# zkeown/mlx-audio-primitives

Measured on AMD Instinct MI355X. Metric: mel-spectrogram frames/sec (n_fft=2048, n_mels=128), higher is better.
Workload: dtype f32

## Files before the change

### mlx-audio-primitives_amd/csrc/ap_launch.h

```cpp
#pragma once
#include <cstdio>

#include <cstdlib>
#include "../../include/audioprims.h"
#include "ap_common.h"
#include "ap_wave_params.h"

char *ap_error_buffer();

#define AP_FAIL(code, ...)                                         \
    do {                                                           \
        std::snprintf(ap_error_buffer(), 512, __VA_ARGS__);        \
        return (code);                                             \
    } while (0)

static const int64_t kApMaxGrid = 2147483647LL;
static const int64_t kApStreamGrid = 256 * 8;

static inline int ap_grid_1d(int64_t total, int block, int64_t cap) {
    int64_t g = (total + block - 1) / block;
    if (g < 1) g = 1;
    if (g > cap) g = cap;
    return (int)g;
}
// ... 220 lines not shown
                                     const int32_t *desc, int n_waves, int x_complex, int partial_off,
                                     int *n_pass, int *grid) {
    if (P.n_mels > 128 || desc[12] > 256 || desc[15] > 4) return 1;
    if (P.T > (1 << 24) || P.L > (1 << 28)) return 1;
    W.y = P.y;
    W.window = P.window;
    W.tw = P.tw;
    W.parts = plan + desc[11];
    W.n_parts = desc[12];
    W.quads = reinterpret_cast<const float *>(plan + desc[13]);
    W.n_quads = desc[14];
    W.n_slots = desc[7];
    W.hopj = P.hop == 512 ? 4 : 0;
    W.max_row_parts = desc[15];
    W.partial_stride = 0;
    if (partial_off + W.n_slots + 4 > 2 * x_complex || partial_off + 64 > 2 * x_complex) return 1;
    W.rowstart = plan + desc[10];
    W.out = P.out_mel;
    W.max_key = nullptr;
    W.L = P.L;
    W.T = P.T;
    W.Ts = P.T;
    W.tiles_per_clip = 0;
    W.n_tiles = 0;
    W.n_clips = B;
    W.hop = P.hop;
    W.pad = P.pad;
    W.pad_mode = P.pad_mode;
    W.n_mels = P.n_mels;
    W.power = P.power;
    const int pass = (W.n_parts + 63) / 64;
    if (pass < 1 || pass > 4 || W.n_quads < 256 * pass) return 1;
    *n_pass = pass;
    int off = n_waves * x_complex * (int)sizeof(ap_float2);
    W.off_tw2 = off; off += APM_TW2_COMPLEX * (int)sizeof(ap_float2);
    W.off_tw1 = off; off += APM_TW1_COMPLEX * (int)sizeof(ap_float2);
    W.off_win = off; off += APW_NC * (int)sizeof(ap_float2);
    W.off_wq = off; off += ap_align16(W.n_quads * 16);
    W.off_parts = off;
    W.off_partial = 0;
    W.off_otile = 0;
    W.otile_stride = 0;
    W.lds_bytes = off;
    if (off > AP_LDS_MAX) return 1;
    const int64_t n_frames = B * P.T;
    int64_t g = (n_frames + (int64_t)n_waves * 8 - 1) / ((int64_t)n_waves * 8);
    if (g > 256) g = 256;
    if (g < 1) g = 1;
    *grid = (int)g;
    return AP_OK;
}

static inline int ap_prepare_spec_run(ApSpecWaveParams &W, const ApStftParams &P, int64_t B, int n_waves,
                                      int x_complex, int *grid) {
    if (P.plan.n != 2048 || !ap_clip_loads_ok(P)) return 1;
    if (P.T > (1 << 24) || P.L > (1 << 28)) return 1;
    W.y = P.y;
    W.window = P.window;
    W.tw = P.tw;
    W.L = P.L;
    W.T = P.T;
    W.n_clips = B;
    W.hop = P.hop;
    W.pad = P.pad;
    W.hopj = P.hop == 512 ? 4 : 0;
    int off = n_waves * x_complex * (int)sizeof(ap_float2);
    W.off_tw2 = off; off += APM_TW2_COMPLEX * (int)sizeof(ap_float2);
    W.off_tw1 = off; off += APM_TW1_COMPLEX * (int)sizeof(ap_float2);
    W.off_win = off; off += APW_NC * (int)sizeof(ap_float2);
    W.lds_bytes = off;
// ... 691 lines not shown
```

### mlx-audio-primitives_amd/csrc/ap_wave_params.h

```cpp
#pragma once
#include "ap_common.h"

#define APW_NC 1024
#define APW_G 8
#define APW_WAVES 8
#define APW_T1(r) ((r) * 20 + ((r) >> 4) * 2)
#define APW_X_COMPLEX 1284
#define APW_PASSES 4
#define APW_TW2_COMPLEX 72
#define APM_TW_ROW 18
#define APM_TW2_ROW 14
#define APM_TW1_COMPLEX (64 * APM_TW_ROW)
#define APM_TW2_COMPLEX (64 * APM_TW2_ROW)

struct ApMelWaveParams {
    const float *y;
    const float *window;
    const ap_float2 *tw;
    const int32_t *parts;
    const float *quads;
    const int32_t *rowstart;
    float *out;
    unsigned *max_key;
    int64_t L, T, tiles_per_clip, n_tiles, n_clips;
    int64_t Ts;
    int hop, pad, pad_mode, n_mels, n_parts, n_quads, n_slots;
    int hopj;
    int max_row_parts;
    int partial_stride;
    float power;
    int off_tw2, off_tw1, off_win, off_wq, off_parts, off_partial, off_otile, lds_bytes;
    int otile_stride;
};

struct ApSpecWaveParams {
    const float *y;
    const float *window;
    const ap_float2 *tw;
    const float *freq;
    float *centroid, *bandwidth, *rolloff, *flatness;
    int64_t L, T, n_clips;
    int hop, pad, hopj, norm;
    float power, p, roll_percent, amin;
    int off_tw2, off_tw1, off_win, lds_bytes;
};

#define APS_WAVES 8
#define APS_OB_ROW 9
#define APS_OB_ROWS 257

struct ApStftWaveParams {
    const float *y;
    const float *window;
    const ap_float2 *tw;
    ap_float2 *out;
    int64_t L, T, groups_per_clip, n_groups;
    int hop, pad, pad_mode;
    int off_tw2, off_tw1, off_win, off_ob, lds_bytes;
};

#define APS16_G 16
// ... 42 lines not shown
```

### mlx-audio-primitives_amd/csrc/audioprims.hip

```cpp
#include <hip/hip_runtime.h>
#include <cstdlib>
#include <mutex>

#include <cstdio>
#include <cstring>

#include "ap_launch.h"
#include "ap_tu.h"
#include "kernels_generic.h"
#include "kernels_wave.h"
#include "kernels_pointwise.h"
#include "kernels_bigfft.h"
#include "kernels_ct.h"
#include "kernels_wave512.h"
#include "kernels_mel2048.h"
#include "kernels_frames8.h"
#include "kernels_features.h"

static thread_local char g_err[512] = "";

char *ap_error_buffer() { return g_err; }

void ap_set_error(const char *msg) { std::snprintf(g_err, sizeof(g_err), "%s", msg); }

static int ap_check_launch(const char *what) {
    hipError_t e = hipGetLastError();
    if (e != hipSuccess) AP_FAIL(AP_ERR_HIP, "%s: %s", what, hipGetErrorString(e));
    return AP_OK;
}

template <class K>
static int ap_allow_lds(K kernel, int bytes) {
    if (bytes > 48 * 1024) {
        hipError_t e = hipFuncSetAttribute(reinterpret_cast<const void *>(kernel),
                                           hipFuncAttributeMaxDynamicSharedMemorySize, bytes);
        if (e != hipSuccess)
            AP_FAIL(AP_ERR_HIP, "hipFuncSetAttribute(LDS=%d): %s", bytes, hipGetErrorString(e));
    }
    return AP_OK;
}

template <int PMODE, int PADGEN>
static int ap_launch_mel_wave(const ApMelWaveParams &W, int grid, void *stream) {
    int rc = ap_allow_lds(ap_mel2048_wave_kernel<PMODE, PADGEN>, W.lds_bytes);
    if (rc != AP_OK) return rc;
    hipLaunchKernelGGL((ap_mel2048_wave_kernel<PMODE, PADGEN>), dim3(grid), dim3(64 * APW_WAVES), W.lds_bytes,
                       (hipStream_t)stream, W);
    return ap_check_launch("ap_melspec_f32(wave)");
}

template <int PMODE, int HOPJ, int IN16>
static int ap_launch_mel_run_h(const ApMelWaveParams &W, int n_pass, int grid, void *stream) {
#define AP_RUN_LAUNCH(NP)                                                                                \
    do {                                                                                                 \
        int rc = ap_allow_lds(ap_mel2048_run_kernel<PMODE, NP, HOPJ, IN16>, W.lds_bytes);                \
        if (rc != AP_OK) return rc;                                                                      \
        hipLaunchKernelGGL((ap_mel2048_run_kernel<PMODE, NP, HOPJ, IN16>), dim3(grid), dim3(64 * APM_WAVES), \
                           W.lds_bytes, (hipStream_t)stream, W);                                         \
    } while (0)
    if (n_pass == 1) AP_RUN_LAUNCH(1);
    else if (n_pass == 2) AP_RUN_LAUNCH(2);
    else if (n_pass == 3) AP_RUN_LAUNCH(3);
    else AP_RUN_LAUNCH(4);
#undef AP_RUN_LAUNCH
    return ap_check_launch("ap_melspec_f32(run)");
}
template <int PMODE, int IN16 = 0>
static int ap_launch_mel_run(const ApMelWaveParams &W, int n_pass, int grid, void *stream) {
    return W.hopj == 4 ? ap_launch_mel_run_h<PMODE, 4, IN16>(W, n_pass, grid, stream)
                       : ap_launch_mel_run_h<PMODE, 0, IN16>(W, n_pass, grid, stream);
}

static const unsigned kApKeyMinusInf = 0x007FFFFFu;

template <int EPI, int PADGEN>
static int ap_launch_ct(ApStftParams &P, int n_fft, int64_t B, void *stream, bool *handled) {
    *handled = false;
    if (P.L > (1 << 28)) return AP_OK;
    int G = 0, lds = 0;
    *handled = false;
    if (!ap_ct_config(n_fft, EPI == 1 ? P.n_parts : 0, EPI == 1 ? P.n_quads : 0, P.n_mels, &G, &lds)) return AP_OK;
    P.tiles_per_clip = (P.T + G - 1) / G;
    int64_t tiles = P.tiles_per_clip * B;
    const int per_cu = AP_LDS_MAX / lds < 8 ? AP_LDS_MAX / lds : 8;
    int64_t grid = tiles < 256 * per_cu ? tiles : 256 * per_cu;
    int rc = AP_OK;
#define AP_CT_LAUNCH(NC, R0, R1, R2, GG, NT)                                                             \
    do {                                                                                                 \
        rc = ap_allow_lds(ap_stft_ct_kernel<EPI, NC, R0, R1, R2, GG, PADGEN, NT>, lds);                  \
        if (rc != AP_OK) return rc;                                                                      \
        hipLaunchKernelGGL((ap_stft_ct_kernel<EPI, NC, R0, R1, R2, GG, PADGEN, NT>), dim3((unsigned)grid), \
                           dim3(NT), lds, (hipStream_t)stream, P);                                       \
    } while (0)
    if (n_fft == 400) AP_CT_LAUNCH(200, 8, 5, 5, 8, 256);
    else if (n_fft == 512) AP_CT_LAUNCH(256, 16, 16, 1, 8, 256);
    else AP_CT_LAUNCH(512, 16, 8, 4, 8, 256);
#undef AP_CT_LAUNCH
// ... 1210 lines not shown
```

### mlx-audio-primitives_amd/csrc/host_builders.cpp

```cpp
#include <algorithm>
#include <cmath>
#include <cstring>
#include <string>
#include <vector>

#include "../../include/audioprims.h"
#include "ap_common.h"

void ap_set_error(const char *msg);

namespace {

const double kPi = 3.14159265358979323846;

const double F_MIN = 0.0;
const double F_SP = 200.0 / 3.0;
const double MIN_LOG_HZ = 1000.0;
const double MIN_LOG_MEL = (MIN_LOG_HZ - F_MIN) / F_SP;
const double LOGSTEP = std::log(6.4) / 27.0;

double hz_to_mel1(double f, int htk) {
    if (htk) return 2595.0 * std::log10(1.0 + f / 700.0);
    if (f < MIN_LOG_HZ) return (f - F_MIN) / F_SP;
    return MIN_LOG_MEL + std::log(f / MIN_LOG_HZ) / LOGSTEP;
// ... 150 lines not shown
        for (int k = 0; k < F; ++k)
            if (fb[(size_t)m * F + k] != 0.0f) { if (!any) a = k; b = k + 1; any = true; }
        if (!any) continue;
        lo[m] = a;
        len[m] = b - a;
        const int gfirst = a >> 2, glast = (b - 1) >> 2;
        for (int g = gfirst; g <= glast; g += 4) {
            MelPart p;
            p.row = m;
            p.g0 = g;
            p.ng = (glast - g + 1) < 4 ? (glast - g + 1) : 4;
            p.q0 = 0;
            p.slot = (int)parts.size();
            parts.push_back(p);
        }
    }
    std::stable_sort(parts.begin(), parts.end(),
                     [](const MelPart &x, const MelPart &y) { return x.ng > y.ng; });
    int q = 0;
    for (auto &p : parts) { p.q0 = q; q += p.ng; }
}

struct MelWaveLayout {
    std::vector<int> partA, partB;
    int n_quads = 0;
};

const int kB128Groups[4][16] = {
    {0, 1, 2, 3, 12, 13, 14, 15, 20, 21, 22, 23, 24, 25, 26, 27},
    {4, 5, 6, 7, 8, 9, 10, 11, 16, 17, 18, 19, 28, 29, 30, 31},
    {32, 33, 34, 35, 44, 45, 46, 47, 52, 53, 54, 55, 56, 57, 58, 59},
    {36, 37, 38, 39, 40, 41, 42, 43, 48, 49, 50, 51, 60, 61, 62, 63}};

void mel_wave_layout(const std::vector<MelPart> &parts, MelWaveLayout &L) {
    std::vector<std::pair<int, int>> ent;
    size_t i = 0;
    for (; i < parts.size() && parts[i].ng > 2; ++i) ent.push_back({(int)i, -1});
    for (; i < parts.size(); i += 2) ent.push_back({(int)i, i + 1 < parts.size() ? (int)i + 1 : -1});
    const int n = (int)ent.size();
    const int passes = (n + 63) / 64;
    L.partA.assign((size_t)passes * 64, -1);
    L.partB.assign((size_t)passes * 64, -1);
    for (int ps = 0; ps < passes; ++ps) {
        const int first = ps * 64, last = first + 64 < n ? first + 64 : n;
        std::vector<int> bucket[16];
        for (int e = first; e < last; ++e) bucket[parts[ent[e].first].g0 & 15].push_back(e);
        int order[16];
        for (int r = 0; r < 16; ++r) order[r] = r;
        std::stable_sort(order, order + 16, [&](int a, int b) { return bucket[a].size() > bucket[b].size(); });
        std::vector<int> grp[4];
        int has[4][16] = {};
        for (int oi = 0; oi < 16; ++oi) {
            const int r = order[oi];
            for (int idx : bucket[r]) {
                int best = -1;
                for (int g = 0; g < 4; ++g) {
                    if (grp[g].size() >= 16) continue;
                    if (best < 0 || has[g][r] < has[best][r] ||
                        (has[g][r] == has[best][r] && grp[g].size() < grp[best].size()))
                        best = g;
                }
                grp[best].push_back(idx);
                has[best][r]++;
            }
        }
        for (int g = 0; g < 4; ++g)
            for (size_t j = 0; j < grp[g].size(); ++j) {
                const size_t slot = (size_t)ps * 64 + kB128Groups[g][j];
                L.partA[slot] = ent[grp[g][j]].first;
                L.partB[slot] = ent[grp[g][j]].second;
            }
    }
    L.n_quads = passes * 256;
}
}

int64_t ap_mel_plan_words(const float *fb, int n_mels, int n_bins) {
    if (!fb || n_mels <= 0 || n_bins <= 0) return 0;
    std::vector<int> lo, len;
    std::vector<MelPart> parts;
    mel_analyse(fb, n_mels, n_bins, lo, len, parts);
    int64_t quads = 0;
    for (auto &p : parts) quads += p.ng;
    MelWaveLayout L;
    mel_wave_layout(parts, L);
    return 2 * (int64_t)n_mels + 4 * (int64_t)parts.size() + 4 * quads + (int64_t)n_mels + 1 + 8 +
           4 * (int64_t)L.partA.size() + 4 * (int64_t)L.n_quads + 8;
}

int ap_mel_plan_host(const float *fb, int n_mels, int n_bins, int32_t *plan, int32_t *desc) {
    if (!fb || !plan || !desc || n_mels <= 0 || n_bins <= 0) {
        ap_set_error("mel plan: bad arguments");
        return AP_ERR_INVALID;
    }
    const int M = n_mels, F = n_bins;
    std::vector<int> lo, len;
    std::vector<MelPart> parts;
    mel_analyse(fb, M, F, lo, len, parts);
    int64_t quads = 0;
    for (auto &p : parts) quads += p.ng;
    const int64_t words = ap_mel_plan_words(fb, M, F);
    std::memset(plan, 0, sizeof(int32_t) * (size_t)words);
    std::memset(desc, 0, sizeof(int32_t) * AP_PLAN_DESC_INTS);
    int64_t off = 0;
    const int64_t off_lo = off; off += M;
    const int64_t off_len = off; off += M;
    off += off & 3 ? 4 - (off & 3) : 0;
    const int64_t off_parts = off; off += 4 * (int64_t)parts.size();
    const int64_t off_quads = off; off += 4 * quads;
    const int64_t off_rs = off; off += (int64_t)M + 1;
    off += off & 3 ? 4 - (off & 3) : 0;
    MelWaveLayout WL;
    mel_wave_layout(parts, WL);
    const int64_t off_wparts = off; off += 4 * (int64_t)WL.partA.size();
    const int64_t off_wquads = off; off += 4 * (int64_t)WL.n_quads;
    for (int m = 0; m < M; ++m) { plan[off_lo + m] = lo[m]; plan[off_len + m] = len[m]; }
    bool parts_ok = true;
    {
        std::vector<int> cnt(M, 0);
        for (auto &p : parts) cnt[p.row]++;
        int acc = 0;
        for (int m = 0; m < M; ++m) { plan[off_rs + m] = acc; acc += cnt[m]; }
        plan[off_rs + M] = acc;
    }
    float *wq = reinterpret_cast<float *>(plan + off_quads);
    for (size_t i = 0; i < parts.size(); ++i) {
        const MelPart &p = parts[i];
        plan[off_parts + 4 * i + 0] = p.slot;
        plan[off_parts + 4 * i + 1] = p.g0;
        plan[off_parts + 4 * i + 2] = p.ng;
        plan[off_parts + 4 * i + 3] = p.q0;
        for (int g = 0; g < p.ng; ++g)
            for (int e = 0; e < 4; ++e) {
                const int k = 4 * (p.g0 + g) + e;
                wq[4 * (size_t)(p.q0 + g) + e] = k < F ? fb[(size_t)p.row * F + k] : 0.0f;
            }
    }
    float *wwq = reinterpret_cast<float *>(plan + off_wquads);
    int max_row_parts = 0;
    for (int m = 0; m < M; ++m)
        if (plan[off_rs + m + 1] - plan[off_rs + m] > max_row_parts)
            max_row_parts = plan[off_rs + m + 1] - plan[off_rs + m];
    const int32_t dump = (int32_t)parts.size();
    auto put_rows = [&](size_t e, int row0, const MelPart &p, int g_first, int g_count) {
        const size_t col = (e / 64) * 256 + (e % 64);
        for (int g = 0; g < g_count; ++g)
// ... 108 lines not shown
```

### mlx-audio-primitives_amd/csrc/kernels_mel2048.h

```cpp
#pragma once
#include <type_traits>
#include "kernels_wave.h"

#define APM_WAVES 8
#define APM_RUN 8
#define APM_PARTIAL_OFF 1152

#define APM_REG_WIN 1
#define APM_REG_TW1 2
#define APM_REG_TW2 4
#define APM_REG_SPLIT 8
#define APM_REGS (APM_REG_WIN | APM_REG_SPLIT)

AP_DEV int apm_gidx(int g) { return 4 * g + 2 * (g >> 3); }

struct ApmPairLane {
    int L, lp;
    bool l0;
    int rd[4];
};

AP_DEV ApmPairLane apm_pair_lane_init(int lane) {
    ApmPairLane p;
    p.L = apm_lane_index(lane);
// ... 47 lines not shown
        const int a = lane & 3, bq = lane >> 2;
#pragma unroll
        for (int k = 0; k < 16; ++k) X[APW_T1(k * 4 + a) + bq] = v[k];
    }
    AP_WAVE_SYNC();
#pragma unroll
    for (int i = 0; i < 16; ++i) v[i] = X[APW_T1(lane) + i];
    AP_WAVE_SYNC();
    ApButterfly<16>::run_twiddled_fused(v, t1, v);
    if (REGS & APM_REG_TW2) {
#pragma unroll
        for (int i = 0; i < 12; ++i) t2[i] = t2r[i];
    } else {
        apm_load_row(tw2row, t2);
    }
    const int wb = apm_gidx(c.k1p) + (lane & 3);
#pragma unroll
    for (int cc = 0; cc < 16; ++cc) X[wb + 68 * cc] = v[cc];
    AP_WAVE_SYNC();
}

AP_DEV void apm_pair_bins(const ApmPairLane &p, int (&k)[8]) {
    k[0] = p.L; k[1] = p.L + 256; k[2] = 512 - p.lp; k[3] = 256 - p.lp;
    k[4] = p.L + 64; k[5] = p.L + 320; k[6] = 448 - p.L; k[7] = 192 - p.L;
}

AP_DEV void apm_split_twiddles(const ApmPairLane &p, const ap_float2 *tw, ap_float2 (&wsp)[8]) {
    int k[8];
    apm_pair_bins(p, k);
#pragma unroll
    for (int i = 0; i < 8; ++i) wsp[i] = ap_scale(tw[k[i]], 0.5f);
}

template <int PMODE>
AP_DEV void apm_split(const ap_float2 *X, float *pp, const ApmPairLane &p, const ap_float2 (&wsp)[8],
                      const ap_float2 (&t2)[12], const ApwLane &c, float power) {
    ap_float2 z[4][4];
#pragma unroll
    for (int s = 0; s < 4; ++s) {
        const ap_float4 *src = reinterpret_cast<const ap_float4 *>(X + p.rd[s]);
        const ap_float4 lo = src[0], hi = src[1];
        z[s][0] = ap_mk(lo.x, lo.y); z[s][1] = ap_mk(lo.z, lo.w);
        z[s][2] = ap_mk(hi.x, hi.y); z[s][3] = ap_mk(hi.z, hi.w);
    }
    AP_WAVE_SYNC();
#pragma unroll
    for (int s = 0; s < 4; ++s)
        ap_fft4_twiddled3(z[s][0], z[s][1], t2[3 * s], z[s][2], t2[3 * s + 1], z[s][3], t2[3 * s + 2]);
    const ap_float2 zk[8] = {z[0][0], z[0][1], z[3][1], z[3][0], z[1][0], z[1][1], z[2][1], z[2][0]};
    const ap_float2 zm[8] = {p.l0 ? z[0][0] : z[3][3], p.l0 ? z[0][3] : z[3][2], p.l0 ? z[3][2] : z[0][2],
                             p.l0 ? z[3][3] : z[0][3], z[2][3], z[2][2], z[1][2], z[1][3]};
    int k[8];
    apm_pair_bins(p, k);
#pragma unroll
    for (int i = 0; i < 8; ++i) {
        const ap_float2 a = ap_add_conj(zk[i], zm[i]);
        const ap_float2 d = ap_sub_conj(zk[i], zm[i]);
        const ap_float2 u = ap_mul_fw(d, wsp[i]);
        const ap_float2 xk = ap_fma_add_mi(a, c.half, u);
        const ap_float2 xm = ap_fma_sub_mi(a, c.half, u);
        pp[k[i]] = apw_pow2x<PMODE>(xk.x, xk.y, power);
        pp[APW_NC - k[i]] = apw_pow2x<PMODE>(xm.x, xm.y, power);
    }
    if (p.l0) pp[APW_NC / 2] = apw_pow2x<PMODE>(z[0][2].x, z[0][2].y, power);
}

#ifdef AP_DIAG_STAMPS
#define AP_DIAG_BEGIN() unsigned long long ap_dt0, ap_dr0; \
    asm volatile("s_memtime %0\n\ts_memrealtime %1\n\ts_waitcnt lgkmcnt(0)" : "=s"(ap_dt0), "=s"(ap_dr0)::"memory")
#define AP_DIAG_END(widx) do { unsigned long long ap_dt1, ap_dr1; \
    asm volatile("s_memtime %0\n\ts_memrealtime %1\n\ts_waitcnt lgkmcnt(0)" : "=s"(ap_dt1), "=s"(ap_dr1)::"memory"); \
    if ((threadIdx.x & 63) == 0 && (widx) < 256 * 16) { ap_diag_stamps[4 * (widx)] = ap_dt1 - ap_dt0; ap_diag_stamps[4 * (widx) + 1] = ap_dr1 - ap_dr0; ap_diag_stamps[4 * (widx) + 2] = ap_dr0; ap_diag_stamps[4 * (widx) + 3] = ap_dr1; } } while (0)
#else
#define AP_DIAG_BEGIN() do {} while (0)
#define AP_DIAG_END(widx) do {} while (0)
#endif

#ifdef AP_HOST_EMU
#define AP_FAIR_SHARE(wave, nw, f) do {} while (0)
#else
#define AP_FAIR_SHARE(wave, nw, f)                                   \
    do {                                                             \
        if ((wave) >= (nw) / 2 + ((nw) > 8 ? 2 : 0)) {               \
            if ((f) & 1) __builtin_amdgcn_s_setprio(1);              \
            else __builtin_amdgcn_s_setprio(0);                      \
        } else if ((nw) > 8 && (wave) >= 4) {                        \
            if ((f) & 1) __builtin_amdgcn_s_setprio(0);              \
            else __builtin_amdgcn_s_setprio(1);                      \
        }                                                            \
    } while (0)
#endif

template <int PMODE, int NPASS, int HOPJ, int IN16 = 0, int NW = APM_WAVES, int REGS = APM_REGS>
__global__ void __launch_bounds__(64 * NW, NW / 4) ap_mel2048_run_kernel(ApMelWaveParams P) {
    static_assert(IN16 != 1 || (REGS & APM_REG_WIN), "the PCM scale rides on the register-resident window");
    const int tid = threadIdx.x;
    const int lane = tid & 63;
    const int wave = AP_UNIFORM(tid >> 6);
    ap_float2 *X = reinterpret_cast<ap_float2 *>(ap_smem) + wave * APW_X_COMPLEX;
    ap_float2 *TW2 = reinterpret_cast<ap_float2 *>(ap_smem + P.off_tw2);
    const ap_float2 *TW1 = reinterpret_cast<const ap_float2 *>(ap_smem + P.off_tw1);
    const ap_float2 *WIN = reinterpret_cast<const ap_float2 *>(ap_smem + P.off_win);
    const ap_float4 *WQ = reinterpret_cast<const ap_float4 *>(ap_smem + P.off_wq);
    float *pp = reinterpret_cast<float *>(X);
    float *partial = pp + APM_PARTIAL_OFF;
    const int M = P.n_mels;

    {
        const int nt = 64 * NW;
        ap_float4 *wq = reinterpret_cast<ap_float4 *>(ap_smem + P.off_wq);
        for (int i = tid; i < P.n_quads; i += nt) wq[i] = reinterpret_cast<const ap_float4 *>(P.quads)[i];
        apm_fill_tables(TW2, reinterpret_cast<ap_float2 *>(ap_smem + P.off_tw1),
                        reinterpret_cast<ap_float2 *>(ap_smem + P.off_win), P.tw, P.window, tid, nt);
    }
    AP_LDS_BARRIER();
    const ApwLane lc = apw_lane_init(lane, TW2, P.tw, APM_TW_ROW);
    const ApmPairLane pl = apm_pair_lane_init(lane);
    ap_float2 winr[16], t1r[16], t2r[12], wsp[8];
#pragma unroll
    for (int j = 0; j < 16; ++j) {
        winr[j] = (REGS & APM_REG_WIN) ? reinterpret_cast<const ap_float2 *>(P.window)[lane + 64 * j] : ap_mk(0.0f, 0.0f);
        if (IN16 == 1) winr[j] = ap_scale(winr[j], 1.0f / 32768.0f);
        t1r[j] = (REGS & APM_REG_TW1) ? P.tw[2 * (4 * j + (lane & 3)) * (lane >> 2)] : ap_mk(0.0f, 0.0f);
        if (j < 12)
            t2r[j] = (REGS & APM_REG_TW2) ? P.tw[32 * (j % 3 + 1) * (apm_lane_group(pl.L, j / 3) >> 4)] : ap_mk(0.0f, 0.0f);
    }
    apm_split_twiddles(pl, P.tw, wsp);
    const ap_float4 *pqa[NPASS], *pqb[NPASS];
    float *sa[NPASS], *sb[NPASS];
    float fz[NPASS];
#pragma unroll
    for (int ps = 0; ps < NPASS; ++ps) {
        const int pi = lane + 64 * ps;
        ap_int4 pd;
        pd.x = P.n_slots; pd.y = 0; pd.z = P.n_slots; pd.w = 0;
        if (pi < P.n_parts) pd = reinterpret_cast<const ap_int4 *>(P.parts)[pi];
        pqa[ps] = reinterpret_cast<const ap_float4 *>(pp) + pd.y;
        pqb[ps] = reinterpret_cast<const ap_float4 *>(pp) + pd.w;
        sa[ps] = partial + pd.x;
        sb[ps] = partial + (pd.z < 0 ? P.n_slots : pd.z);
        fz[ps] = pd.z < 0 ? 1.0f : 0.0f;
    }
    int rs0[2], cnt[2];
#pragma unroll
    for (int i = 0; i < 2; ++i) {
        const int row = lane + 64 * i;
        rs0[i] = row < M ? P.rowstart[row] : 0;
        cnt[i] = row < M ? P.rowstart[row + 1] - rs0[i] : 0;
    }
    AP_LDS_BARRIER();

    const int64_t worker = (int64_t)blockIdx.x * NW + wave;
    const int64_t n_workers = (int64_t)gridDim.x * NW;
    const int64_t n_frames = P.n_clips * P.T;
    const int64_t f_lo = n_frames * worker / n_workers, f_hi = n_frames * (worker + 1) / n_workers;
    const int Ti = (int)P.T;
    float vmax = -INFINITY;
    AP_DIAG_BEGIN();
    if (f_lo < f_hi) {
        int64_t b = f_lo / P.T;
        int t = (int)(f_lo - b * P.T);
        const int16_t *y16 = reinterpret_cast<const int16_t *>(P.y);
        ApClip clip = ap_clip_make(P.y + (IN16 == 1 ? 0 : b * P.L), IN16 == 1 ? 0 : P.L);
        ApClip16 clip16 = ap_clip16_make(y16 + (IN16 == 1 ? b * P.L : 0), IN16 == 1 ? P.L : 0);
        auto ld2 = [&](int64_t bb, int base, int p) -> ap_float2 {
            if (IN16 == 1) return ap_clip16_load2(clip16, p);
            if (IN16 == 2 && !(base >= 0 && (int64_t)base + 2 * APW_NC <= P.L)) {
                const float *yb = P.y + bb * P.L;
                return ap_mk(ap_load_padded(yb, P.L, p, P.pad_mode), ap_load_padded(yb, P.L, p + 1, P.pad_mode));
            }
            return ap_clip_load2(clip, p);
        };
        constexpr int U = HOPJ == 4 ? 4 : 1;
        ap_float2 raw[16];
        auto load_frame = [&](int tt, auto rot_tag) {
            constexpr int ROT = decltype(rot_tag)::value;
            const int base = tt * P.hop - P.pad;
#pragma unroll
            for (int j = 0; j < 16; ++j) {
                const int p = base + 2 * (lane + 64 * j);
                raw[(j + HOPJ * ROT) & 15] = ld2(b, base, p);
            }
        };
        const int r0 = U == 4 ? (t & 3) : 0;
        if (r0 == 1) load_frame(t, std::integral_constant<int, 1 % U>());
        else if (r0 == 2) load_frame(t, std::integral_constant<int, 2 % U>());
        else if (r0 == 3) load_frame(t, std::integral_constant<int, 3 % U>());
        else load_frame(t, std::integral_constant<int, 0>());
        float acc0[APM_RUN], acc1[APM_RUN];
#pragma unroll
        for (int i = 0; i < APM_RUN; ++i) { acc0[i] = 0.0f; acc1[i] = 0.0f; }
        int nrun = 0, half = U == 4 ? ((t >> 2) & 1) : 0;
        int64_t f = f_lo;

        auto frame = [&](auto rot_tag) -> bool {
            constexpr int ROT = decltype(rot_tag)::value;
            constexpr int NROT = (ROT + 1) % U;
            AP_FAIR_SHARE(wave, NW, f);
            const bool clip_ends = t + 1 == Ti;
            const bool more = f + 1 < f_hi;
            ap_float2 t2[12];
            {
                ap_float2 xs[16], ws[16];
#pragma unroll
                for (int j = 0; j < 16; ++j) xs[j] = raw[(j + HOPJ * ROT) & 15];
                if (REGS & APM_REG_WIN) {
#pragma unroll
                    for (int j = 0; j < 16; ++j) ws[j] = winr[j];
                } else {
#pragma unroll
                    for (int j = 0; j < 16; ++j) ws[j] = WIN[lane + 64 * j];
                }
                AP_SCHED_FENCE();
                apm_forward<REGS>(xs, ws, X, TW1 + APM_TW_ROW * lane, TW2 + APM_TW2_ROW * lane, t1r, t2r, t2, lc);
            }
            AP_SCHED_FENCE();
            if (more) {
                if (clip_ends) {
                    if (IN16 == 1) clip16 = ap_clip16_make(y16 + (b + 1) * P.L, P.L);
                    else clip = ap_clip_make(P.y + (b + 1) * P.L, P.L);
                }
                const int base = (clip_ends ? 0 : t + 1) * P.hop - P.pad;
#pragma unroll
                for (int j = 16 - HOPJ; j < 16; ++j) {
                    const int p = base + 2 * (lane + 64 * j);
                    raw[(j + HOPJ * NROT) & 15] = ld2(clip_ends ? b + 1 : b, base, p);
                }
                if (HOPJ == 0 || clip_ends) {
#pragma unroll
                    for (int j = 0; j < 16 - HOPJ; ++j) {
                        const int p = base + 2 * (lane + 64 * j);
                        raw[(j + HOPJ * NROT) & 15] = ld2(clip_ends ? b + 1 : b, base, p);
                    }
                }
            }
            AP_SCHED_FENCE();
            apm_split<PMODE>(X, pp, pl, wsp, t2, lc, P.power);
            AP_WAVE_SYNC();
#pragma unroll
            for (int ps = 0; ps < NPASS; ++ps) {
                const ap_float4 *wq = WQ + 256 * ps + lane;
                ap_float4 w[4], q[4];
#pragma unroll
                for (int i = 0; i < 4; ++i) w[i] = wq[64 * i];
                q[0] = pqa[ps][0]; q[1] = pqa[ps][1]; q[2] = pqb[ps][0]; q[3] = pqb[ps][1];
                float acc[2] = {0.0f, 0.0f};
#pragma unroll
                for (int i = 0; i < 4; ++i) {
                    acc[i >> 1] = fmaf(w[i].x, q[i].x, acc[i >> 1]);
                    acc[i >> 1] = fmaf(w[i].y, q[i].y, acc[i >> 1]);
                    acc[i >> 1] = fmaf(w[i].z, q[i].z, acc[i >> 1]);
                    acc[i >> 1] = fmaf(w[i].w, q[i].w, acc[i >> 1]);
                }
                *sa[ps] = fmaf(fz[ps], acc[1], acc[0]);
                *sb[ps] = acc[1];
            }
            AP_WAVE_SYNC();
            float sum2[2];
#pragma unroll
            for (int i = 0; i < 2; ++i) {
                const float p0 = partial[rs0[i]], p1 = partial[rs0[i] + 1], p2 = partial[rs0[i] + 2],
                            p3 = partial[rs0[i] + 3];
                float sum = cnt[i] > 0 ? p0 : 0.0f;
                sum += cnt[i] > 1 ? p1 : 0.0f;
                sum += cnt[i] > 2 ? p2 : 0.0f;
                sum += cnt[i] > 3 ? p3 : 0.0f;
                sum2[i] = sum;
                vmax = fmaxf(vmax, cnt[i] > 0 ? sum : vmax);
            }
            int pos;
            if (U == 1) {
#pragma unroll
                for (int i = 0; i < APM_RUN - 1; ++i) { acc0[i] = acc0[i + 1]; acc1[i] = acc1[i + 1]; }
                acc0[APM_RUN - 1] = sum2[0];
                acc1[APM_RUN - 1] = sum2[1];
                pos = APM_RUN - 1;
            } else {
                if (half) { acc0[4 + ROT] = sum2[0]; acc1[4 + ROT] = sum2[1]; }
                else { acc0[ROT] = sum2[0]; acc1[ROT] = sum2[1]; }
                pos = 4 * half + ROT;
            }
            ++nrun;
            AP_WAVE_SYNC();
            if ((U == 1 ? nrun == APM_RUN : pos == APM_RUN - 1) || clip_ends || !more) {
                const int first = pos - nrun + 1;
                float *ob = P.out + b * (int64_t)M * P.Ts + (t - nrun + 1);
#pragma unroll
                for (int i = 0; i < 2; ++i) {
                    const int row = lane + 64 * i;
                    if (row < M) {
                        float *dst = ob + (int64_t)row * P.Ts;
                        const float *src = i == 0 ? acc0 : acc1;
                        if (nrun == APM_RUN) {
                            ap_rsp_f4u lo, hi;
                            lo.x = src[0]; lo.y = src[1]; lo.z = src[2]; lo.w = src[3];
                            hi.x = src[4]; hi.y = src[5]; hi.z = src[6]; hi.w = src[7];
                            *reinterpret_cast<ap_rsp_f4u *>(dst) = lo;
                            *reinterpret_cast<ap_rsp_f4u *>(dst + 4) = hi;
                        } else {
#pragma unroll
                            for (int g = 0; g < APM_RUN; ++g)
                                if (g >= first && g <= pos) dst[g - first] = src[g];
                        }
                    }
                }
                nrun = 0;
            }
            if (clip_ends) { t = 0; ++b; } else { ++t; }
            ++f;
            return more;
        };
        if (U == 1) {
            while (frame(std::integral_constant<int, 0>())) {}
        } else {
            int skip = r0;
            for (;;) {
                if (skip <= 0 && !frame(std::integral_constant<int, 0>())) break;
                if (skip <= 1 && !frame(std::integral_constant<int, 1 % U>())) break;
                if (skip <= 2 && !frame(std::integral_constant<int, 2 % U>())) break;
                if (!frame(std::integral_constant<int, 3 % U>())) break;
                skip = 0;
                half ^= 1;
            }
        }
    }
    AP_DIAG_END((int)worker);
    if (P.max_key) {
        AP_WAVE_SYNC();
        partial[lane] = vmax;
        AP_WAVE_SYNC();
        if (lane == 0) {
            float m = partial[0];
            for (int i = 1; i < 64; ++i) m = fmaxf(m, partial[i]);
            ap_atomic_max_u32(P.max_key, ap_fkey(m));
        }
    }
}

#ifdef AP_HOST_EMU
AP_DEV float apm_lane_xor(float x, int mask) { return emu_lane_xor(x, mask); }
AP_DEV float apm_lane_up(float x, int d, int lane) { return emu_lane_perm(x, lane - d); }
#else
// ... 173 lines not shown
```

### mlx-audio-primitives_amd/csrc/kernels_wave.h

```cpp
#pragma once
#include "ap_wave_params.h"
#include "fft_lds.h"
#include "kernels_generic.h"

#if defined(AP_DIAG_STAMPS) && !defined(AP_HOST_EMU)
__device__ unsigned long long ap_diag_stamps[4 * 256 * 16];
#endif

#define APW_C32(r) ((float)__builtin_cos(6.283185307179586476925 * (r) / 32.0))
#define APW_S32(r) ((float)__builtin_sin(6.283185307179586476925 * (r) / 32.0))

#ifdef AP_HOST_EMU
#define AP_WAVE_SYNC() emu_wave_sync()
#define AP_SCHED_FENCE() do {} while (0)
#define AP_PIN(x) do {} while (0)
#else
#define AP_SCHED_FENCE() __builtin_amdgcn_sched_barrier(0)
#define AP_PIN(x) asm volatile("" : "+v"(x))
#define AP_WAVE_SYNC()                                          \
    do {                                                        \
        __builtin_amdgcn_fence(__ATOMIC_RELEASE, "wavefront");  \
        __builtin_amdgcn_wave_barrier();                        \
        __builtin_amdgcn_fence(__ATOMIC_ACQUIRE, "wavefront");  \
    } while (0)
// ... 104 lines not shown
    c.halfc = ap_mk(0.5f, -0.5f);
    return c;
}

template <bool QUAD_SIGNS = true>
AP_DEV void apw_fill_tables(ap_float2 *tw2, ap_float2 *tw1, ap_float2 *win, const ap_float2 *tw,
                            const float *window, int tid, int nt) {
    if (tid < 64) {
        const int a = tid >> 4;
        tw2[a * 17 + (tid & 15)] = ap_scale(tw[32 * a * (tid & 15)], (QUAD_SIGNS && (a == 1 || a == 2)) ? -1.0f : 1.0f);
    }
    for (int i = tid; i < 16 * 64; i += nt) tw1[i] = tw[2 * (i & 63) * (i >> 6)];
    for (int i = tid; i < APW_NC; i += nt) win[i] = reinterpret_cast<const ap_float2 *>(window)[i];
}

AP_DEV int apm_lane_index(int lane) {
    return (int)((0xE311825200ull >> (5 * ((lane >> 2) & 7))) & 31) + (lane & 3) + (lane & 32);
}
AP_DEV int apm_lane_group(int L, int s) {
    return s == 0 ? L : s == 1 ? L + 64 : s == 2 ? 192 - L : 256 - (L == 0 ? 128 : L);
}

AP_DEV void apm_fill_tables(ap_float2 *tw2, ap_float2 *tw1, ap_float2 *win, const ap_float2 *tw,
                            const float *window, int tid, int nt) {
    for (int i = tid; i < APM_TW2_COMPLEX; i += nt) {
        const int l = i / APM_TW2_ROW, e = i % APM_TW2_ROW;
        const int c = apm_lane_group(apm_lane_index(l), e / 3) >> 4, a = e % 3 + 1;
        tw2[i] = e < 12 ? tw[32 * a * c] : ap_mk(0.0f, 0.0f);
    }
    for (int i = tid; i < APM_TW1_COMPLEX; i += nt) {
        const int l = i / APM_TW_ROW, e = i % APM_TW_ROW;
        tw1[i] = e < 16 ? tw[2 * (4 * e + (l & 3)) * (l >> 2)] : ap_mk(0.0f, 0.0f);
    }
    for (int i = tid; i < APW_NC; i += nt) win[i] = reinterpret_cast<const ap_float2 *>(window)[i];
}

struct ApmLane {
    float c1, c2;
    float sg;
    bool rot;
};

AP_DEV ApmLane apm_lane_init(int lane) {
    ApmLane m;
    const int qa = lane & 3;
    const float s1 = qa < 2 ? 1.0f : -1.0f, s2 = (qa & 1) ? -1.0f : 1.0f;
    m.c1 = -s1;
    m.c2 = -s2;
    m.sg = s1 * s2;
    m.rot = qa == 3;
    return m;
}

#ifdef AP_HOST_EMU
AP_DEV void apm_quad8(ap_float2 *v, const ApmLane &m) {
    for (int i = 0; i < 8; ++i) {
        v[i].x = v[i].x + m.c1 * ap_quad_xor2(v[i].x);
        v[i].y = v[i].y + m.c1 * ap_quad_xor2(v[i].y);
    }
    for (int i = 0; i < 8; ++i) {
        const float rx = v[i].x, ry = v[i].y;
        v[i].x = m.rot ? ry : rx;
        v[i].y = m.rot ? -rx : ry;
    }
    for (int i = 0; i < 8; ++i) {
        v[i].x = v[i].x + m.c2 * ap_quad_xor1(v[i].x);
// ... 728 lines not shown
```

Baseline: 662.7 million.

## Pair consecutive frames in mel contraction and reorder filterbank parts to cut bank conflicts

For hop-512 runs, the kernel parks the power spectrum of the even rotation in an extra per-wave LDS plane. The next frame's contraction then processes both frames together, so each mel-weight quad is loaded once for two frames and partial sums are stored as float2 pairs. Host plan building gains a local-search swap pass that reorders part assignments across lane groups to lower LDS bank conflicts. The window table is dropped from LDS to make room. The cost is more LDS per wave, which may reduce occupancy, plus added branching and code size.

New measurement: 674.8 million, median of 6. +1.8%, better.

```diff
diff --git a/mlx-audio-primitives_amd/csrc/ap_launch.h b/mlx-audio-primitives_amd/csrc/ap_launch.h
--- a/mlx-audio-primitives_amd/csrc/ap_launch.h
+++ b/mlx-audio-primitives_amd/csrc/ap_launch.h
@@ -276,10 +276,14 @@
     const int pass = (W.n_parts + 63) / 64;
     if (pass < 1 || pass > 4 || W.n_quads < 256 * pass) return 1;
     *n_pass = pass;
-    int off = n_waves * x_complex * (int)sizeof(ap_float2);
+    const int tables = (APM_TW2_COMPLEX + APM_TW1_COMPLEX + (APM_MEL_WIN_LDS ? APW_NC : 0)) * (int)sizeof(ap_float2) +
+                       ap_align16(W.n_quads * 16);
+    W.pair = W.hopj == 4 && partial_off + 2 * (W.n_slots + 4) <= 2 * x_complex &&
+             n_waves * (x_complex + APM_PARK_COMPLEX) * (int)sizeof(ap_float2) + tables <= AP_LDS_MAX;
+    int off = n_waves * (x_complex + (W.pair ? APM_PARK_COMPLEX : 0)) * (int)sizeof(ap_float2);
     W.off_tw2 = off; off += APM_TW2_COMPLEX * (int)sizeof(ap_float2);
     W.off_tw1 = off; off += APM_TW1_COMPLEX * (int)sizeof(ap_float2);
-    W.off_win = off; off += APW_NC * (int)sizeof(ap_float2);
+    W.off_win = off; off += APM_MEL_WIN_LDS ? APW_NC * (int)sizeof(ap_float2) : 0;
     W.off_wq = off; off += ap_align16(W.n_quads * 16);
     W.off_parts = off;
     W.off_partial = 0;
diff --git a/mlx-audio-primitives_amd/csrc/ap_wave_params.h b/mlx-audio-primitives_amd/csrc/ap_wave_params.h
--- a/mlx-audio-primitives_amd/csrc/ap_wave_params.h
+++ b/mlx-audio-primitives_amd/csrc/ap_wave_params.h
@@ -12,6 +12,8 @@
 #define APM_TW2_ROW 14
 #define APM_TW1_COMPLEX (64 * APM_TW_ROW)
 #define APM_TW2_COMPLEX (64 * APM_TW2_ROW)
+#define APM_PARK_COMPLEX 520
+#define APM_MEL_WIN_LDS 0
 
 struct ApMelWaveParams {
     const float *y;
@@ -27,6 +29,7 @@
     int hop, pad, pad_mode, n_mels, n_parts, n_quads, n_slots;
     int hopj;
     int max_row_parts;
+    int pair;
     int partial_stride;
     float power;
     int off_tw2, off_tw1, off_win, off_wq, off_parts, off_partial, off_otile, lds_bytes;
diff --git a/mlx-audio-primitives_amd/csrc/audioprims.hip b/mlx-audio-primitives_amd/csrc/audioprims.hip
--- a/mlx-audio-primitives_amd/csrc/audioprims.hip
+++ b/mlx-audio-primitives_amd/csrc/audioprims.hip
@@ -51,18 +51,24 @@
 
 template <int PMODE, int HOPJ, int IN16>
 static int ap_launch_mel_run_h(const ApMelWaveParams &W, int n_pass, int grid, void *stream) {
+#define AP_RUN_LAUNCH_P(NP, PAIR)                                                                        \
+    do {                                                                                                 \
+        int rc = ap_allow_lds(ap_mel2048_run_kernel<PMODE, NP, HOPJ, IN16, APM_WAVES, APM_REGS, PAIR>, W.lds_bytes); \
+        if (rc != AP_OK) return rc;                                                                      \
+        hipLaunchKernelGGL((ap_mel2048_run_kernel<PMODE, NP, HOPJ, IN16, APM_WAVES, APM_REGS, PAIR>), dim3(grid), \
+                           dim3(64 * APM_WAVES), W.lds_bytes, (hipStream_t)stream, W);                   \
+    } while (0)
 #define AP_RUN_LAUNCH(NP)                                                                                \
     do {                                                                                                 \
-        int rc = ap_allow_lds(ap_mel2048_run_kernel<PMODE, NP, HOPJ, IN16>, W.lds_bytes);                \
-        if (rc != AP_OK) return rc;                                                                      \
-        hipLaunchKernelGGL((ap_mel2048_run_kernel<PMODE, NP, HOPJ, IN16>), dim3(grid), dim3(64 * APM_WAVES), \
-                           W.lds_bytes, (hipStream_t)stream, W);                                         \
+        if (HOPJ == 4 && W.pair) AP_RUN_LAUNCH_P(NP, (HOPJ == 4));                                       \
+        else AP_RUN_LAUNCH_P(NP, 0);                                                                     \
     } while (0)
     if (n_pass == 1) AP_RUN_LAUNCH(1);
     else if (n_pass == 2) AP_RUN_LAUNCH(2);
     else if (n_pass == 3) AP_RUN_LAUNCH(3);
     else AP_RUN_LAUNCH(4);
 #undef AP_RUN_LAUNCH
+#undef AP_RUN_LAUNCH_P
     return ap_check_launch("ap_melspec_f32(run)");
 }
 template <int PMODE, int IN16 = 0>
diff --git a/mlx-audio-primitives_amd/csrc/host_builders.cpp b/mlx-audio-primitives_amd/csrc/host_builders.cpp
--- a/mlx-audio-primitives_amd/csrc/host_builders.cpp
+++ b/mlx-audio-primitives_amd/csrc/host_builders.cpp
@@ -206,7 +206,21 @@
     {32, 33, 34, 35, 44, 45, 46, 47, 52, 53, 54, 55, 56, 57, 58, 59},
     {36, 37, 38, 39, 40, 41, 42, 43, 48, 49, 50, 51, 60, 61, 62, 63}};
 
-void mel_wave_layout(const std::vector<MelPart> &parts, MelWaveLayout &L) {
+int mel_wave_entries(const std::vector<MelPart> &parts) {
+    int whole = 0;
+    for (auto &p : parts) whole += p.ng > 2;
+    return whole + ((int)parts.size() - whole + 1) / 2;
+}
+
+int64_t mel_plan_words_of(int n_mels, const std::vector<MelPart> &parts) {
+    int64_t quads = 0;
+    for (auto &p : parts) quads += p.ng;
+    const int64_t passes = (mel_wave_entries(parts) + 63) / 64;
+    return 2 * (int64_t)n_mels + 4 * (int64_t)parts.size() + 4 * quads + (int64_t)n_mels + 1 + 8 +
+           4 * 64 * passes + 4 * 256 * passes + 8;
+}
+
+void mel_wave_layout(const std::vector<MelPart> &parts, bool n2048, MelWaveLayout &L) {
     std::vector<std::pair<int, int>> ent;
     size_t i = 0;
     for (; i < parts.size() && parts[i].ng > 2; ++i) ent.push_back({(int)i, -1});
@@ -245,6 +259,59 @@
                 L.partB[slot] = ent[grp[g][j]].second;
             }
     }
+    if (n2048 && passes <= 4) {
+        const int n_pos = passes * 64;
+        auto groups_of = [&](int pos, int &gA, int &gB) {
+            gA = gB = 0;
+            if (L.partA[pos] < 0) return;
+            gA = parts[L.partA[pos]].g0;
+            gB = L.partB[pos] >= 0 ? parts[L.partB[pos]].g0 : gA + 2;
+        };
+        auto cost_of = [&](int ps, int g, int &worst, int &squares) {
+            worst = 0; squares = 0;
+            for (int half = 0; half < 2; ++half) {
+                int seen[16][16], n_seen[16] = {};
+                for (int j = 0; j < 16; ++j) {
+                    int gA, gB;
+                    groups_of(ps * 64 + kB128Groups[g][j], gA, gB);
+                    const int grp = half ? gB : gA, r = grp & 15;
+                    bool dup = false;
+                    for (int k = 0; k < n_seen[r]; ++k) dup = dup || seen[r][k] == grp;
+                    if (!dup) seen[r][n_seen[r]++] = grp;
+                }
+                int m = 0;
+                for (int r = 0; r < 16; ++r) { if (n_seen[r] > m) m = n_seen[r]; squares += n_seen[r] * n_seen[r]; }
+                worst += m;
+            }
+        };
+        int lane_group[64];
+        for (int g = 0; g < 4; ++g)
+            for (int j = 0; j < 16; ++j) lane_group[kB128Groups[g][j]] = g;
+        std::vector<int> cw((size_t)passes * 4), cs((size_t)passes * 4);
+        for (int ps = 0; ps < passes; ++ps)
+            for (int g = 0; g < 4; ++g) cost_of(ps, g, cw[ps * 4 + g], cs[ps * 4 + g]);
+        for (int sweep = 0, improved = 1; improved && sweep < 16; ++sweep) {
+            improved = 0;
+            for (int i = 0; i < n_pos; ++i)
+                for (int j = i + 1; j < n_pos; ++j) {
+                    const int ki = (i / 64) * 4 + lane_group[i % 64], kj = (j / 64) * 4 + lane_group[j % 64];
+                    if (ki == kj) continue;
+                    std::swap(L.partA[i], L.partA[j]);
+                    std::swap(L.partB[i], L.partB[j]);
+                    int wi, si, wj, sj;
+                    cost_of(ki / 4, ki % 4, wi, si);
+                    cost_of(kj / 4, kj % 4, wj, sj);
+                    const int dw = wi + wj - cw[ki] - cw[kj], dsq = si + sj - cs[ki] - cs[kj];
+                    if (dw < 0 || (dw == 0 && dsq < 0)) {
+                        cw[ki] = wi; cs[ki] = si; cw[kj] = wj; cs[kj] = sj;
+                        improved = 1;
+                    } else {
+                        std::swap(L.partA[i], L.partA[j]);
+                        std::swap(L.partB[i], L.partB[j]);
+                    }
+                }
+        }
+    }
     L.n_quads = passes * 256;
 }
 }
@@ -254,12 +321,7 @@
     std::vector<int> lo, len;
     std::vector<MelPart> parts;
     mel_analyse(fb, n_mels, n_bins, lo, len, parts);
-    int64_t quads = 0;
-    for (auto &p : parts) quads += p.ng;
-    MelWaveLayout L;
-    mel_wave_layout(parts, L);
-    return 2 * (int64_t)n_mels + 4 * (int64_t)parts.size() + 4 * quads + (int64_t)n_mels + 1 + 8 +
-           4 * (int64_t)L.partA.size() + 4 * (int64_t)L.n_quads + 8;
+    return mel_plan_words_of(n_mels, parts);
 }
 
 int ap_mel_plan_host(const float *fb, int n_mels, int n_bins, int32_t *plan, int32_t *desc) {
@@ -273,7 +335,7 @@
     mel_analyse(fb, M, F, lo, len, parts);
     int64_t quads = 0;
     for (auto &p : parts) quads += p.ng;
-    const int64_t words = ap_mel_plan_words(fb, M, F);
+    const int64_t words = mel_plan_words_of(M, parts);
     std::memset(plan, 0, sizeof(int32_t) * (size_t)words);
     std::memset(desc, 0, sizeof(int32_t) * AP_PLAN_DESC_INTS);
     int64_t off = 0;
@@ -285,7 +347,7 @@
     const int64_t off_rs = off; off += (int64_t)M + 1;
     off += off & 3 ? 4 - (off & 3) : 0;
     MelWaveLayout WL;
-    mel_wave_layout(parts, WL);
+    mel_wave_layout(parts, F == 1025, WL);
     const int64_t off_wparts = off; off += 4 * (int64_t)WL.partA.size();
     const int64_t off_wquads = off; off += 4 * (int64_t)WL.n_quads;
     for (int m = 0; m < M; ++m) { plan[off_lo + m] = lo[m]; plan[off_len + m] = len[m]; }
diff --git a/mlx-audio-primitives_amd/csrc/kernels_mel2048.h b/mlx-audio-primitives_amd/csrc/kernels_mel2048.h
--- a/mlx-audio-primitives_amd/csrc/kernels_mel2048.h
+++ b/mlx-audio-primitives_amd/csrc/kernels_mel2048.h
@@ -103,7 +103,7 @@
     for (int i = 0; i < 8; ++i) wsp[i] = ap_scale(tw[k[i]], 0.5f);
 }
 
-template <int PMODE>
+template <int PMODE, int POFF = 0>
 AP_DEV void apm_split(const ap_float2 *X, float *pp, const ApmPairLane &p, const ap_float2 (&wsp)[8],
                       const ap_float2 (&t2)[12], const ApwLane &c, float power) {
     ap_float2 z[4][4];
@@ -130,10 +130,10 @@
         const ap_float2 u = ap_mul_fw(d, wsp[i]);
         const ap_float2 xk = ap_fma_add_mi(a, c.half, u);
         const ap_float2 xm = ap_fma_sub_mi(a, c.half, u);
-        pp[k[i]] = apw_pow2x<PMODE>(xk.x, xk.y, power);
-        pp[APW_NC - k[i]] = apw_pow2x<PMODE>(xm.x, xm.y, power);
-    }
-    if (p.l0) pp[APW_NC / 2] = apw_pow2x<PMODE>(z[0][2].x, z[0][2].y, power);
+        pp[k[i] + POFF] = apw_pow2x<PMODE>(xk.x, xk.y, power);
+        pp[APW_NC - k[i] + POFF] = apw_pow2x<PMODE>(xm.x, xm.y, power);
+    }
+    if (p.l0) pp[APW_NC / 2 + POFF] = apw_pow2x<PMODE>(z[0][2].x, z[0][2].y, power);
 }
 
 #ifdef AP_DIAG_STAMPS
@@ -162,13 +162,32 @@
     } while (0)
 #endif
 
-template <int PMODE, int NPASS, int HOPJ, int IN16 = 0, int NW = APM_WAVES, int REGS = APM_REGS>
+#ifdef AP_PACKED_COMPLEX
+AP_DEV ap_float4 apm_load4(const ap_float4 *p) {
+    const apm_float4v v = *reinterpret_cast<const apm_float4v *>(p);
+    ap_float4 r;
+    r.x = v.x; r.y = v.y; r.z = v.z; r.w = v.w;
+    return r;
+}
+#else
+AP_DEV ap_float4 apm_load4(const ap_float4 *p) { return *p; }
+#endif
+
+template <int PMODE, int NPASS, int HOPJ, int IN16 = 0, int NW = APM_WAVES, int REGS = APM_REGS, int PAIR = (HOPJ == 4)>
 __global__ void __launch_bounds__(64 * NW, NW / 4) ap_mel2048_run_kernel(ApMelWaveParams P) {
     static_assert(IN16 != 1 || (REGS & APM_REG_WIN), "the PCM scale rides on the register-resident window");
+    static_assert(APM_MEL_WIN_LDS || (REGS & APM_REG_WIN), "ap_prepare_mel_run leaves no room for a window table");
+    static_assert(!PAIR || HOPJ == 4, "pairs are two of the four rotations of the hop-512 loop");
+    constexpr int XS = APW_X_COMPLEX + (PAIR ? APM_PARK_COMPLEX : 0);
+    constexpr int SS = PAIR ? 2 : 1;
+    static_assert(2 * APM_PARK_COMPLEX >= 4 * (APW_NC / 4 + 4), "groups 256 .. 259: the contraction's read-ahead");
+#ifdef AP_HOST_EMU
+    if ((PAIR != 0) != (P.pair != 0)) { fprintf(stderr, "ap_mel2048_run_kernel: PAIR = %d on a carve-up for pair = %d\n", PAIR, P.pair); abort(); }
+#endif
     const int tid = threadIdx.x;
     const int lane = tid & 63;
     const int wave = AP_UNIFORM(tid >> 6);
-    ap_float2 *X = reinterpret_cast<ap_float2 *>(ap_smem) + wave * APW_X_COMPLEX;
+    ap_float2 *X = reinterpret_cast<ap_float2 *>(ap_smem) + wave * XS;
     ap_float2 *TW2 = reinterpret_cast<ap_float2 *>(ap_smem + P.off_tw2);
     const ap_float2 *TW1 = reinterpret_cast<const ap_float2 *>(ap_smem + P.off_tw1);
     const ap_float2 *WIN = reinterpret_cast<const ap_float2 *>(ap_smem + P.off_win);
@@ -182,7 +201,8 @@
         ap_float4 *wq = reinterpret_cast<ap_float4 *>(ap_smem + P.off_wq);
         for (int i = tid; i < P.n_quads; i += nt) wq[i] = reinterpret_cast<const ap_float4 *>(P.quads)[i];
         apm_fill_tables(TW2, reinterpret_cast<ap_float2 *>(ap_smem + P.off_tw1),
-                        reinterpret_cast<ap_float2 *>(ap_smem + P.off_win), P.tw, P.window, tid, nt);
+                        (REGS & APM_REG_WIN) ? nullptr : reinterpret_cast<ap_float2 *>(ap_smem + P.off_win),
+                        P.tw, P.window, tid, nt);
     }
     AP_LDS_BARRIER();
     const ApwLane lc = apw_lane_init(lane, TW2, P.tw, APM_TW_ROW);
@@ -208,9 +228,12 @@
         if (pi < P.n_parts) pd = reinterpret_cast<const ap_int4 *>(P.parts)[pi];
         pqa[ps] = reinterpret_cast<const ap_float4 *>(pp) + pd.y;
         pqb[ps] = reinterpret_cast<const ap_float4 *>(pp) + pd.w;
-        sa[ps] = partial + pd.x;
-        sb[ps] = partial + (pd.z < 0 ? P.n_slots : pd.z);
+        sa[ps] = partial + SS * pd.x;
+        sb[ps] = partial + SS * (pd.z < 0 ? P.n_slots : pd.z);
         fz[ps] = pd.z < 0 ? 1.0f : 0.0f;
+    }
+    if (PAIR) {
+        for (int i = APW_NC + 1 + lane; i < 2 * APM_PARK_COMPLEX; i += 64) pp[2 * APW_X_COMPLEX + i] = 0.0f;
     }
     int rs0[2], cnt[2];
 #pragma unroll
@@ -218,6 +241,7 @@
         const int row = lane + 64 * i;
         rs0[i] = row < M ? P.rowstart[row] : 0;
         cnt[i] = row < M ? P.rowstart[row + 1] - rs0[i] : 0;
+        rs0[i] *= SS;
     }
     AP_LDS_BARRIER();
 
@@ -234,7 +258,7 @@
         const int16_t *y16 = reinterpret_cast<const int16_t *>(P.y);
         ApClip clip = ap_clip_make(P.y + (IN16 == 1 ? 0 : b * P.L), IN16 == 1 ? 0 : P.L);
         ApClip16 clip16 = ap_clip16_make(y16 + (IN16 == 1 ? b * P.L : 0), IN16 == 1 ? P.L : 0);
-        auto ld2 = [&](int64_t bb, int base, int p) -> ap_float2 {
+        auto ld2 = [&](int64_t bb, int base, int p) __attribute__((always_inline)) -> ap_float2 {
             if (IN16 == 1) return ap_clip16_load2(clip16, p);
             if (IN16 == 2 && !(base >= 0 && (int64_t)base + 2 * APW_NC <= P.L)) {
                 const float *yb = P.y + bb * P.L;
@@ -264,12 +288,10 @@
         int nrun = 0, half = U == 4 ? ((t >> 2) & 1) : 0;
         int64_t f = f_lo;
 
-        auto frame = [&](auto rot_tag) -> bool {
+        auto transform = [&](auto rot_tag, auto poff_tag, const bool clip_ends, const bool more) __attribute__((always_inline)) {
             constexpr int ROT = decltype(rot_tag)::value;
             constexpr int NROT = (ROT + 1) % U;
             AP_FAIR_SHARE(wave, NW, f);
-            const bool clip_ends = t + 1 == Ti;
-            const bool more = f + 1 < f_hi;
             ap_float2 t2[12];
             {
                 ap_float2 xs[16], ws[16];
@@ -306,39 +328,11 @@
                 }
             }
             AP_SCHED_FENCE();
-            apm_split<PMODE>(X, pp, pl, wsp, t2, lc, P.power);
+            apm_split<PMODE, decltype(poff_tag)::value>(X, pp, pl, wsp, t2, lc, P.power);
             AP_WAVE_SYNC();
-#pragma unroll
-            for (int ps = 0; ps < NPASS; ++ps) {
-                const ap_float4 *wq = WQ + 256 * ps + lane;
-                ap_float4 w[4], q[4];
-#pragma unroll
-                for (int i = 0; i < 4; ++i) w[i] = wq[64 * i];
-                q[0] = pqa[ps][0]; q[1] = pqa[ps][1]; q[2] = pqb[ps][0]; q[3] = pqb[ps][1];
-                float acc[2] = {0.0f, 0.0f};
-#pragma unroll
-                for (int i = 0; i < 4; ++i) {
-                    acc[i >> 1] = fmaf(w[i].x, q[i].x, acc[i >> 1]);
-                    acc[i >> 1] = fmaf(w[i].y, q[i].y, acc[i >> 1]);
-                    acc[i >> 1] = fmaf(w[i].z, q[i].z, acc[i >> 1]);
-                    acc[i >> 1] = fmaf(w[i].w, q[i].w, acc[i >> 1]);
-                }
-                *sa[ps] = fmaf(fz[ps], acc[1], acc[0]);
-                *sb[ps] = acc[1];
-            }
-            AP_WAVE_SYNC();
-            float sum2[2];
-#pragma unroll
-            for (int i = 0; i < 2; ++i) {
-                const float p0 = partial[rs0[i]], p1 = partial[rs0[i] + 1], p2 = partial[rs0[i] + 2],
-                            p3 = partial[rs0[i] + 3];
-                float sum = cnt[i] > 0 ? p0 : 0.0f;
-                sum += cnt[i] > 1 ? p1 : 0.0f;
-                sum += cnt[i] > 2 ? p2 : 0.0f;
-                sum += cnt[i] > 3 ? p3 : 0.0f;
-                sum2[i] = sum;
-                vmax = fmaxf(vmax, cnt[i] > 0 ? sum : vmax);
-            }
+        };
+        auto finish = [&](auto rot_tag, const float (&sum2)[2], const bool clip_ends, const bool more) __attribute__((always_inline)) {
+            constexpr int ROT = decltype(rot_tag)::value;
             int pos;
             if (U == 1) {
 #pragma unroll
@@ -379,6 +373,106 @@
             }
             if (clip_ends) { t = 0; ++b; } else { ++t; }
             ++f;
+        };
+        constexpr int PARKQ = 2 * APW_X_COMPLEX / 4;
+        static_assert(2 * APW_X_COMPLEX % 4 == 0 && (APW_X_COMPLEX + APM_PARK_COMPLEX) % 2 == 0, "16-byte aligned planes");
+        auto contract = [&](auto pq_tag, float (&sum2)[2]) __attribute__((always_inline)) {
+            constexpr int PQ = decltype(pq_tag)::value;
+#pragma unroll
+            for (int ps = 0; ps < NPASS; ++ps) {
+                const ap_float4 *wq = WQ + 256 * ps + lane;
+                ap_float4 w[4], q[4];
+#pragma unroll
+                for (int i = 0; i < 4; ++i) w[i] = wq[64 * i];
+                q[0] = pqa[ps][PQ]; q[1] = pqa[ps][PQ + 1]; q[2] = pqb[ps][PQ]; q[3] = pqb[ps][PQ + 1];
+                float acc[2] = {0.0f, 0.0f};
+#pragma unroll
+                for (int i = 0; i < 4; ++i) {
+                    acc[i >> 1] = fmaf(w[i].x, q[i].x, acc[i >> 1]);
+                    acc[i >> 1] = fmaf(w[i].y, q[i].y, acc[i >> 1]);
+                    acc[i >> 1] = fmaf(w[i].z, q[i].z, acc[i >> 1]);
+                    acc[i >> 1] = fmaf(w[i].w, q[i].w, acc[i >> 1]);
+                }
+                *sa[ps] = fmaf(fz[ps], acc[1], acc[0]);
+                *sb[ps] = acc[1];
+            }
+            AP_WAVE_SYNC();
+#pragma unroll
+            for (int i = 0; i < 2; ++i) {
+                const float p0 = partial[rs0[i]], p1 = partial[rs0[i] + SS], p2 = partial[rs0[i] + 2 * SS],
+                            p3 = partial[rs0[i] + 3 * SS];
+                float sum = cnt[i] > 0 ? p0 : 0.0f;
+                sum += cnt[i] > 1 ? p1 : 0.0f;
+                sum += cnt[i] > 2 ? p2 : 0.0f;
+                sum += cnt[i] > 3 ? p3 : 0.0f;
+                sum2[i] = sum;
+                vmax = fmaxf(vmax, cnt[i] > 0 ? sum : vmax);
+            }
+        };
+        auto contract_pair = [&](float (&sum0)[2], float (&sum1)[2]) __attribute__((always_inline)) {
+#pragma unroll
+            for (int ps = 0; ps < NPASS; ++ps) {
+                const ap_float4 *wq = WQ + 256 * ps + lane;
+                ap_float4 w[4], q0[4], q1[4];
+#pragma unroll
+                for (int i = 0; i < 4; ++i) w[i] = apm_load4(wq + 64 * i);
+                q0[0] = apm_load4(pqa[ps] + PARKQ); q0[1] = apm_load4(pqa[ps] + PARKQ + 1);
+                q0[2] = apm_load4(pqb[ps] + PARKQ); q0[3] = apm_load4(pqb[ps] + PARKQ + 1);
+                q1[0] = apm_load4(pqa[ps]); q1[1] = apm_load4(pqa[ps] + 1);
+                q1[2] = apm_load4(pqb[ps]); q1[3] = apm_load4(pqb[ps] + 1);
+                float a0[2] = {0.0f, 0.0f}, a1[2] = {0.0f, 0.0f};
+#pragma unroll
+                for (int i = 0; i < 4; ++i) {
+                    a0[i >> 1] = fmaf(w[i].x, q0[i].x, a0[i >> 1]);
+                    a0[i >> 1] = fmaf(w[i].y, q0[i].y, a0[i >> 1]);
+                    a0[i >> 1] = fmaf(w[i].z, q0[i].z, a0[i >> 1]);
+                    a0[i >> 1] = fmaf(w[i].w, q0[i].w, a0[i >> 1]);
+                    a1[i >> 1] = fmaf(w[i].x, q1[i].x, a1[i >> 1]); AP_PIN(a1[i >> 1]);
+                    a1[i >> 1] = fmaf(w[i].y, q1[i].y, a1[i >> 1]); AP_PIN(a1[i >> 1]);
+                    a1[i >> 1] = fmaf(w[i].z, q1[i].z, a1[i >> 1]); AP_PIN(a1[i >> 1]);
+                    if (i < 3) { a1[i >> 1] = fmaf(w[i].w, q1[i].w, a1[i >> 1]); AP_PIN(a1[i >> 1]); }
+                }
+                float s0 = fmaf(fz[ps], a0[1], a0[0]);
+                AP_PIN(s0);
+                a1[1] = fmaf(w[3].w, q1[3].w, a1[1]); AP_PIN(a1[1]);
+                *reinterpret_cast<ap_float2 *>(sa[ps]) = ap_mk(s0, fmaf(fz[ps], a1[1], a1[0]));
+                *reinterpret_cast<ap_float2 *>(sb[ps]) = ap_mk(a0[1], a1[1]);
+            }
+            AP_WAVE_SYNC();
+#pragma unroll
+            for (int i = 0; i < 2; ++i) {
+                const ap_float2 *pr = reinterpret_cast<const ap_float2 *>(partial + rs0[i]);
+                const ap_float2 p0 = pr[0], p1 = pr[1], p2 = pr[2], p3 = pr[3];
+                float s0 = cnt[i] > 0 ? p0.x : 0.0f, s1 = cnt[i] > 0 ? p0.y : 0.0f;
+                s0 += cnt[i] > 1 ? p1.x : 0.0f; s1 += cnt[i] > 1 ? p1.y : 0.0f;
+                s0 += cnt[i] > 2 ? p2.x : 0.0f; s1 += cnt[i] > 2 ? p2.y : 0.0f;
+                s0 += cnt[i] > 3 ? p3.x : 0.0f; s1 += cnt[i] > 3 ? p3.y : 0.0f;
+                sum0[i] = s0; sum1[i] = s1;
+                vmax = fmaxf(vmax, cnt[i] > 0 ? fmaxf(s0, s1) : vmax);
+            }
+        };
+        bool paired = false;
+        auto frame = [&](auto rot_tag) __attribute__((always_inline)) -> bool {
+            constexpr int ROT = decltype(rot_tag)::value;
+            constexpr bool FIRST = PAIR && ROT % 2 == 0;
+            const bool clip_ends = t + 1 == Ti;
+            const bool more = f + 1 < f_hi;
+            transform(rot_tag, std::integral_constant<int, FIRST ? 4 * PARKQ : 0>(), clip_ends, more);
+            float sum2[2];
+            if (FIRST) {
+                paired = !clip_ends && more;
+                sum2[0] = sum2[1] = 0.0f;
+                if (!paired) contract(std::integral_constant<int, PARKQ>(), sum2);
+            } else if (PAIR && paired) {
+                float sum0[2];
+                contract_pair(sum0, sum2);
+                if (half) { acc0[4 + (ROT + 3) % 4] = sum0[0]; acc1[4 + (ROT + 3) % 4] = sum0[1]; }
+                else { acc0[(ROT + 3) % 4] = sum0[0]; acc1[(ROT + 3) % 4] = sum0[1]; }
+                paired = false;
+            } else {
+                contract(std::integral_constant<int, 0>(), sum2);
+            }
+            finish(rot_tag, sum2, clip_ends, more);
             return more;
         };
         if (U == 1) {
diff --git a/mlx-audio-primitives_amd/csrc/kernels_wave.h b/mlx-audio-primitives_amd/csrc/kernels_wave.h
--- a/mlx-audio-primitives_amd/csrc/kernels_wave.h
+++ b/mlx-audio-primitives_amd/csrc/kernels_wave.h
@@ -160,6 +160,7 @@
         const int l = i / APM_TW_ROW, e = i % APM_TW_ROW;
         tw1[i] = e < 16 ? tw[2 * (4 * e + (l & 3)) * (l >> 2)] : ap_mk(0.0f, 0.0f);
     }
+    if (!win) return;
     for (int i = tid; i < APW_NC; i += nt) win[i] = reinterpret_cast<const ap_float2 *>(window)[i];
 }
 
```
